# PaddlePaddle/PaddleNLP

Measured on NVIDIA H100. Metric: tokens/sec Llama-3.2-3B seq4096 bf16 pretrain step (global, all GPUs), higher is better.
Workload: dtype bf16

## Files before the change

### paddlenlp_b200/csrc/common.cuh

```cuda
#pragma once
#include <cuda.h>
#include <cuda_bf16.h>
#include <cuda_runtime.h>
#include <stdint.h>
#include <stdio.h>

namespace b200 {

typedef __nv_bfloat16 bf16;

__device__ __forceinline__ uint32_t smem_u32(const void* p) {
  return static_cast<uint32_t>(__cvta_generic_to_shared(p));
}
__device__ __forceinline__ void named_bar_sync(uint32_t id, uint32_t nthreads) {
  asm volatile("bar.sync %0, %1;" ::"r"(id), "r"(nthreads) : "memory");
}

__device__ __forceinline__ void pdl_wait() { asm volatile("griddepcontrol.wait;" ::: "memory"); }
__device__ __forceinline__ void pdl_launch_dependents() { asm volatile("griddepcontrol.launch_dependents;" ::: "memory"); }

__device__ __forceinline__ void mbar_init(uint64_t* bar, uint32_t count) {
  asm volatile("mbarrier.init.shared::cta.b64 [%0], %1;" ::"r"(smem_u32(bar)), "r"(count) : "memory");
}
__device__ __forceinline__ void fence_mbar_init() {
// ... 59 lines not shown
                                            int c2, int c3) {
  asm volatile(
      "cp.async.bulk.tensor.4d.shared::cluster.global.mbarrier::complete_tx::bytes [%0], [%1, {%3, %4, %5, %6}], [%2];"
      ::"r"(smem_u32(smem_dst)), "l"(reinterpret_cast<uint64_t>(tm)), "r"(smem_u32(bar)), "r"(c0), "r"(c1), "r"(c2),
      "r"(c3)
      : "memory");
}
__device__ __forceinline__ void tma_reduce_add_4d(const CUtensorMap* tm, const void* smem_src, int c0, int c1, int c2,
                                                  int c3) {
  asm volatile("cp.reduce.async.bulk.tensor.4d.global.shared::cta.add.tile.bulk_group [%0, {%2, %3, %4, %5}], [%1];" ::"l"(
                   reinterpret_cast<uint64_t>(tm)),
               "r"(smem_u32(smem_src)), "r"(c0), "r"(c1), "r"(c2), "r"(c3)
               : "memory");
}
__device__ __forceinline__ void tma_reduce_add_2d(const CUtensorMap* tm, uint32_t smem_src, int c0, int c1) {
  asm volatile("cp.reduce.async.bulk.tensor.2d.global.shared::cta.add.tile.bulk_group [%0, {%2, %3}], [%1];" ::"l"(
                   reinterpret_cast<uint64_t>(tm)),
               "r"(smem_src), "r"(c0), "r"(c1)
               : "memory");
}
__device__ __forceinline__ void tma_store_2d(const CUtensorMap* tm, uint32_t smem_src, int c0, int c1) {
  asm volatile("cp.async.bulk.tensor.2d.global.shared::cta.bulk_group [%0, {%2, %3}], [%1];" ::"l"(reinterpret_cast<uint64_t>(tm)),
               "r"(smem_src), "r"(c0), "r"(c1)
               : "memory");
}
__device__ __forceinline__ void tma_prefetch_l2_2d(const CUtensorMap* tm, int c0, int c1) {
  asm volatile("cp.async.bulk.prefetch.tensor.2d.L2.global.tile [%0, {%1, %2}];" ::"l"(reinterpret_cast<uint64_t>(tm)), "r"(c0),
               "r"(c1)
               : "memory");
}
__device__ __forceinline__ void tma_store_commit() { asm volatile("cp.async.bulk.commit_group;" ::: "memory"); }
template <int N>
__device__ __forceinline__ void tma_store_wait_read() {
  asm volatile("cp.async.bulk.wait_group.read %0;" ::"n"(N) : "memory");
}
template <int N>
__device__ __forceinline__ void tma_store_wait() {
  asm volatile("cp.async.bulk.wait_group %0;" ::"n"(N) : "memory");
}

__device__ __forceinline__ uint64_t wgmma_desc_sw128(uint32_t saddr, uint32_t lbo_bytes, uint32_t sbo_bytes) {
  uint64_t d = 0;
  d |= static_cast<uint64_t>((saddr & 0x3FFFFu) >> 4);
  d |= static_cast<uint64_t>((lbo_bytes >> 4) & 0x3FFFu) << 16;
  d |= static_cast<uint64_t>((sbo_bytes >> 4) & 0x3FFFu) << 32;
  d |= static_cast<uint64_t>(1) << 62;
  return d;
}
__device__ __forceinline__ void wgmma_fence() { asm volatile("wgmma.fence.sync.aligned;" ::: "memory"); }
__device__ __forceinline__ void wgmma_commit() { asm volatile("wgmma.commit_group.sync.aligned;" ::: "memory"); }
template <int N>
__device__ __forceinline__ void wgmma_wait() { asm volatile("wgmma.wait_group.sync.aligned %0;" ::"n"(N) : "memory"); }
template <int R>
__device__ __forceinline__ void setmaxnreg_dec() { asm volatile("setmaxnreg.dec.sync.aligned.u32 %0;" ::"n"(R)); }
template <int R>
__device__ __forceinline__ void setmaxnreg_inc() { asm volatile("setmaxnreg.inc.sync.aligned.u32 %0;" ::"n"(R)); }

template <int TA, int TB>
__device__ __forceinline__ void wgmma_m64n256k16(float (&d)[128], uint64_t desc_a, uint64_t desc_b, uint32_t accumulate) {
  asm volatile(
      "{\n\t.reg .pred p;\n\tsetp.ne.b32 p, %130, 0;\n\t"
      "wgmma.mma_async.sync.aligned.m64n256k16.f32.bf16.bf16 "
      "{%0, %1, %2, %3, %4, %5, %6, %7, %8, %9, %10, %11, %12, %13, %14, %15, %16, %17, %18, %19, %20, %21, %22, %23, %24, %25, %26, %27, %28, %29, %30, %31, %32, %33, %34, %35, %36, %37, %38, %39, %40, %41, %42, %43, %44, %45, %46, %47, %48, %49, %50, %51, %52, %53, %54, %55, %56, %57, %58, %59, %60, %61, %62, %63, %64, %65, %66, %67, %68, %69, %70, %71, %72, %73, %74, %75, %76, %77, %78, %79, %80, %81, %82, %83, %84, %85, %86, %87, %88, %89, %90, %91, %92, %93, %94, %95, %96, %97, %98, %99, %100, %101, %102, %103, %104, %105, %106, %107, %108, %109, %110, %111, %112, %113, %114, %115, %116, %117, %118, %119, %120, %121, %122, %123, %124, %125, %126, %127}, %128, %129, p, 1, 1, %131, %132;\n\t}\n"
      : "+f"(d[0]), "+f"(d[1]), "+f"(d[2]), "+f"(d[3]), "+f"(d[4]), "+f"(d[5]), "+f"(d[6]), "+f"(d[7]), "+f"(d[8]), "+f"(d[9]), "+f"(d[10]), "+f"(d[11]), "+f"(d[12]), "+f"(d[13]), "+f"(d[14]), "+f"(d[15]), "+f"(d[16]), "+f"(d[17]), "+f"(d[18]), "+f"(d[19]), "+f"(d[20]), "+f"(d[21]), "+f"(d[22]), "+f"(d[23]), "+f"(d[24]), "+f"(d[25]), "+f"(d[26]), "+f"(d[27]), "+f"(d[28]), "+f"(d[29]), "+f"(d[30]), "+f"(d[31]), "+f"(d[32]), "+f"(d[33]), "+f"(d[34]), "+f"(d[35]), "+f"(d[36]), "+f"(d[37]), "+f"(d[38]), "+f"(d[39]), "+f"(d[40]), "+f"(d[41]), "+f"(d[42]), "+f"(d[43]), "+f"(d[44]), "+f"(d[45]), "+f"(d[46]), "+f"(d[47]), "+f"(d[48]), "+f"(d[49]), "+f"(d[50]), "+f"(d[51]), "+f"(d[52]), "+f"(d[53]), "+f"(d[54]), "+f"(d[55]), "+f"(d[56]), "+f"(d[57]), "+f"(d[58]), "+f"(d[59]), "+f"(d[60]), "+f"(d[61]), "+f"(d[62]), "+f"(d[63]), "+f"(d[64]), "+f"(d[65]), "+f"(d[66]), "+f"(d[67]), "+f"(d[68]), "+f"(d[69]), "+f"(d[70]), "+f"(d[71]), "+f"(d[72]), "+f"(d[73]), "+f"(d[74]), "+f"(d[75]), "+f"(d[76]), "+f"(d[77]), "+f"(d[78]), "+f"(d[79]), "+f"(d[80]), "+f"(d[81]), "+f"(d[82]), "+f"(d[83]), "+f"(d[84]), "+f"(d[85]), "+f"(d[86]), "+f"(d[87]), "+f"(d[88]), "+f"(d[89]), "+f"(d[90]), "+f"(d[91]), "+f"(d[92]), "+f"(d[93]), "+f"(d[94]), "+f"(d[95]), "+f"(d[96]), "+f"(d[97]), "+f"(d[98]), "+f"(d[99]), "+f"(d[100]), "+f"(d[101]), "+f"(d[102]), "+f"(d[103]), "+f"(d[104]), "+f"(d[105]), "+f"(d[106]), "+f"(d[107]), "+f"(d[108]), "+f"(d[109]), "+f"(d[110]), "+f"(d[111]), "+f"(d[112]), "+f"(d[113]), "+f"(d[114]), "+f"(d[115]), "+f"(d[116]), "+f"(d[117]), "+f"(d[118]), "+f"(d[119]), "+f"(d[120]), "+f"(d[121]), "+f"(d[122]), "+f"(d[123]), "+f"(d[124]), "+f"(d[125]), "+f"(d[126]), "+f"(d[127])
      : "l"(desc_a), "l"(desc_b), "r"(accumulate), "n"(TA), "n"(TB));
}
template <int TA, int TB>
__device__ __forceinline__ void wgmma_m64n64k16(float (&d)[32], uint64_t desc_a, uint64_t desc_b, uint32_t accumulate) {
  asm volatile(
      "{\n\t.reg .pred p;\n\tsetp.ne.b32 p, %34, 0;\n\t"
      "wgmma.mma_async.sync.aligned.m64n64k16.f32.bf16.bf16 "
      "{%0, %1, %2, %3, %4, %5, %6, %7, %8, %9, %10, %11, %12, %13, %14, %15, %16, %17, %18, %19, %20, %21, %22, %23, %24, %25, %26, %27, %28, %29, %30, %31}, %32, %33, p, 1, 1, %35, %36;\n\t}\n"
      : "+f"(d[0]), "+f"(d[1]), "+f"(d[2]), "+f"(d[3]), "+f"(d[4]), "+f"(d[5]), "+f"(d[6]), "+f"(d[7]), "+f"(d[8]), "+f"(d[9]), "+f"(d[10]), "+f"(d[11]), "+f"(d[12]), "+f"(d[13]), "+f"(d[14]), "+f"(d[15]), "+f"(d[16]), "+f"(d[17]), "+f"(d[18]), "+f"(d[19]), "+f"(d[20]), "+f"(d[21]), "+f"(d[22]), "+f"(d[23]), "+f"(d[24]), "+f"(d[25]), "+f"(d[26]), "+f"(d[27]), "+f"(d[28]), "+f"(d[29]), "+f"(d[30]), "+f"(d[31])
      : "l"(desc_a), "l"(desc_b), "r"(accumulate), "n"(TA), "n"(TB));
}
template <int TA, int TB>
__device__ __forceinline__ void wgmma_m64n128k16(float (&d)[64], uint64_t desc_a, uint64_t desc_b, uint32_t accumulate) {
  asm volatile(
      "{\n\t.reg .pred p;\n\tsetp.ne.b32 p, %66, 0;\n\t"
      "wgmma.mma_async.sync.aligned.m64n128k16.f32.bf16.bf16 "
      "{%0, %1, %2, %3, %4, %5, %6, %7, %8, %9, %10, %11, %12, %13, %14, %15, %16, %17, %18, %19, %20, %21, %22, %23, %24, %25, %26, %27, %28, %29, %30, %31, %32, %33, %34, %35, %36, %37, %38, %39, %40, %41, %42, %43, %44, %45, %46, %47, %48, %49, %50, %51, %52, %53, %54, %55, %56, %57, %58, %59, %60, %61, %62, %63}, %64, %65, p, 1, 1, %67, %68;\n\t}\n"
      : "+f"(d[0]), "+f"(d[1]), "+f"(d[2]), "+f"(d[3]), "+f"(d[4]), "+f"(d[5]), "+f"(d[6]), "+f"(d[7]), "+f"(d[8]), "+f"(d[9]), "+f"(d[10]), "+f"(d[11]), "+f"(d[12]), "+f"(d[13]), "+f"(d[14]), "+f"(d[15]), "+f"(d[16]), "+f"(d[17]), "+f"(d[18]), "+f"(d[19]), "+f"(d[20]), "+f"(d[21]), "+f"(d[22]), "+f"(d[23]), "+f"(d[24]), "+f"(d[25]), "+f"(d[26]), "+f"(d[27]), "+f"(d[28]), "+f"(d[29]), "+f"(d[30]), "+f"(d[31]), "+f"(d[32]), "+f"(d[33]), "+f"(d[34]), "+f"(d[35]), "+f"(d[36]), "+f"(d[37]), "+f"(d[38]), "+f"(d[39]), "+f"(d[40]), "+f"(d[41]), "+f"(d[42]), "+f"(d[43]), "+f"(d[44]), "+f"(d[45]), "+f"(d[46]), "+f"(d[47]), "+f"(d[48]), "+f"(d[49]), "+f"(d[50]), "+f"(d[51]), "+f"(d[52]), "+f"(d[53]), "+f"(d[54]), "+f"(d[55]), "+f"(d[56]), "+f"(d[57]), "+f"(d[58]), "+f"(d[59]), "+f"(d[60]), "+f"(d[61]), "+f"(d[62]), "+f"(d[63])
      : "l"(desc_a), "l"(desc_b), "r"(accumulate), "n"(TA), "n"(TB));
}
template <int TB>
__device__ __forceinline__ void wgmma_m64n128k16_rs(float (&d)[64], const uint32_t* a, uint64_t desc_b, uint32_t accumulate) {
  asm volatile(
      "{\n\t.reg .pred p;\n\tsetp.ne.b32 p, %69, 0;\n\t"
      "wgmma.mma_async.sync.aligned.m64n128k16.f32.bf16.bf16 "
      "{%0, %1, %2, %3, %4, %5, %6, %7, %8, %9, %10, %11, %12, %13, %14, %15, %16, %17, %18, %19, %20, %21, %22, %23, %24, %25, %26, %27, %28, %29, %30, %31, %32, %33, %34, %35, %36, %37, %38, %39, %40, %41, %42, %43, %44, %45, %46, %47, %48, %49, %50, %51, %52, %53, %54, %55, %56, %57, %58, %59, %60, %61, %62, %63}, {%64, %65, %66, %67}, %68, p, 1, 1, %70;\n\t}\n"
      : "+f"(d[0]), "+f"(d[1]), "+f"(d[2]), "+f"(d[3]), "+f"(d[4]), "+f"(d[5]), "+f"(d[6]), "+f"(d[7]), "+f"(d[8]), "+f"(d[9]), "+f"(d[10]), "+f"(d[11]), "+f"(d[12]), "+f"(d[13]), "+f"(d[14]), "+f"(d[15]), "+f"(d[16]), "+f"(d[17]), "+f"(d[18]), "+f"(d[19]), "+f"(d[20]), "+f"(d[21]), "+f"(d[22]), "+f"(d[23]), "+f"(d[24]), "+f"(d[25]), "+f"(d[26]), "+f"(d[27]), "+f"(d[28]), "+f"(d[29]), "+f"(d[30]), "+f"(d[31]), "+f"(d[32]), "+f"(d[33]), "+f"(d[34]), "+f"(d[35]), "+f"(d[36]), "+f"(d[37]), "+f"(d[38]), "+f"(d[39]), "+f"(d[40]), "+f"(d[41]), "+f"(d[42]), "+f"(d[43]), "+f"(d[44]), "+f"(d[45]), "+f"(d[46]), "+f"(d[47]), "+f"(d[48]), "+f"(d[49]), "+f"(d[50]), "+f"(d[51]), "+f"(d[52]), "+f"(d[53]), "+f"(d[54]), "+f"(d[55]), "+f"(d[56]), "+f"(d[57]), "+f"(d[58]), "+f"(d[59]), "+f"(d[60]), "+f"(d[61]), "+f"(d[62]), "+f"(d[63])
      : "r"(a[0]), "r"(a[1]), "r"(a[2]), "r"(a[3]), "l"(desc_b), "r"(accumulate), "n"(TB));
}
template <int TB>
__device__ __forceinline__ void wgmma_m64n64k16_rs(float (&d)[32], const uint32_t* a, uint64_t desc_b, uint32_t accumulate) {
  asm volatile(
      "{\n\t.reg .pred p;\n\tsetp.ne.b32 p, %37, 0;\n\t"
      "wgmma.mma_async.sync.aligned.m64n64k16.f32.bf16.bf16 "
      "{%0, %1, %2, %3, %4, %5, %6, %7, %8, %9, %10, %11, %12, %13, %14, %15, %16, %17, %18, %19, %20, %21, %22, %23, %24, %25, %26, %27, %28, %29, %30, %31}, {%32, %33, %34, %35}, %36, p, 1, 1, %38;\n\t}\n"
      : "+f"(d[0]), "+f"(d[1]), "+f"(d[2]), "+f"(d[3]), "+f"(d[4]), "+f"(d[5]), "+f"(d[6]), "+f"(d[7]), "+f"(d[8]), "+f"(d[9]), "+f"(d[10]), "+f"(d[11]), "+f"(d[12]), "+f"(d[13]), "+f"(d[14]), "+f"(d[15]), "+f"(d[16]), "+f"(d[17]), "+f"(d[18]), "+f"(d[19]), "+f"(d[20]), "+f"(d[21]), "+f"(d[22]), "+f"(d[23]), "+f"(d[24]), "+f"(d[25]), "+f"(d[26]), "+f"(d[27]), "+f"(d[28]), "+f"(d[29]), "+f"(d[30]), "+f"(d[31])
      : "r"(a[0]), "r"(a[1]), "r"(a[2]), "r"(a[3]), "l"(desc_b), "r"(accumulate), "n"(TB));
}

__device__ __forceinline__ void mma_bf16_16816(float (&c)[4], const uint32_t (&a)[4], uint32_t b0, uint32_t b1) {
  asm volatile(
      "mma.sync.aligned.m16n8k16.row.col.f32.bf16.bf16.f32 {%0, %1, %2, %3}, {%4, %5, %6, %7}, {%8, %9}, "
      "{%0, %1, %2, %3};"
      : "+f"(c[0]), "+f"(c[1]), "+f"(c[2]), "+f"(c[3])
      : "r"(a[0]), "r"(a[1]), "r"(a[2]), "r"(a[3]), "r"(b0), "r"(b1));
}
__device__ __forceinline__ void ldsm_x4(uint32_t saddr, uint32_t (&r)[4]) {
  asm volatile("ldmatrix.sync.aligned.m8n8.x4.shared.b16 {%0, %1, %2, %3}, [%4];"
               : "=r"(r[0]), "=r"(r[1]), "=r"(r[2]), "=r"(r[3])
               : "r"(saddr));
}
__device__ __forceinline__ void ldsm_x4_t(uint32_t saddr, uint32_t (&r)[4]) {
  asm volatile("ldmatrix.sync.aligned.m8n8.x4.trans.shared.b16 {%0, %1, %2, %3}, [%4];"
               : "=r"(r[0]), "=r"(r[1]), "=r"(r[2]), "=r"(r[3])
               : "r"(saddr));
}
__device__ __forceinline__ void cp_async_16(uint32_t saddr, const void* gptr, uint32_t src_bytes) {
  asm volatile("cp.async.cg.shared.global [%0], [%1], 16, %2;" ::"r"(saddr), "l"(gptr), "r"(src_bytes) : "memory");
}
__device__ __forceinline__ void cp_async_commit() { asm volatile("cp.async.commit_group;" ::: "memory"); }
template <int N>
__device__ __forceinline__ void cp_async_wait() { asm volatile("cp.async.wait_group %0;" ::"n"(N) : "memory"); }

__device__ __forceinline__ uint32_t pack_bf16x2(float lo, float hi) {
  __nv_bfloat162 v = __floats2bfloat162_rn(lo, hi);
  return *reinterpret_cast<uint32_t*>(&v);
}
__device__ __forceinline__ float2 unpack_bf16x2(uint32_t u) {
  __nv_bfloat162 v = *reinterpret_cast<__nv_bfloat162*>(&u);
  return __bfloat1622float2(v);
}
__device__ __forceinline__ float bf16_round(float x) { return __bfloat162float(__float2bfloat16_rn(x)); }

__device__ __forceinline__ uint4 ld_nc_v4(const void* p) {
  uint4 r;
  asm("ld.global.nc.L1::no_allocate.v4.u32 {%0, %1, %2, %3}, [%4];"
               : "=r"(r.x), "=r"(r.y), "=r"(r.z), "=r"(r.w)
               : "l"(p));
  return r;
}
__device__ __forceinline__ void st_na_v4(void* p, const uint4& v) {
  asm volatile("st.global.L1::no_allocate.v4.u32 [%0], {%1, %2, %3, %4};" ::"l"(p), "r"(v.x), "r"(v.y), "r"(v.z),
               "r"(v.w));
}
__device__ __forceinline__ void st_shared_u32(uint32_t saddr, uint32_t v) {
  asm volatile("st.shared.u32 [%0], %1;" ::"r"(saddr), "r"(v));
}
__device__ __forceinline__ void st_shared_f32x2(uint32_t saddr, float a, float b) {
  asm volatile("st.shared.v2.f32 [%0], {%1, %2};" ::"r"(saddr), "f"(a), "f"(b));
}
__device__ __forceinline__ uint4 ld_shared_v4(uint32_t saddr) {
  uint4 r;
  asm volatile("ld.shared.v4.u32 {%0, %1, %2, %3}, [%4];" : "=r"(r.x), "=r"(r.y), "=r"(r.z), "=r"(r.w) : "r"(saddr));
  return r;
}

__device__ __forceinline__ float fast_exp2(float x) {
  float y;
  asm("ex2.approx.ftz.f32 %0, %1;" : "=f"(y) : "f"(x));
  return y;
}
__device__ __forceinline__ float fast_rcp(float x) {
  float y;
  asm("rcp.approx.ftz.f32 %0, %1;" : "=f"(y) : "f"(x));
  return y;
}

struct f32x2 { float x, y; };
__device__ __forceinline__ f32x2 f2_mul(f32x2 a, f32x2 b) { return f32x2{__fmul_rn(a.x, b.x), __fmul_rn(a.y, b.y)}; }
__device__ __forceinline__ f32x2 f2_add(f32x2 a, f32x2 b) { return f32x2{__fadd_rn(a.x, b.x), __fadd_rn(a.y, b.y)}; }
__device__ __forceinline__ f32x2 f2_fma(f32x2 a, f32x2 b, f32x2 c) {
  return f32x2{__fmaf_rn(a.x, b.x, c.x), __fmaf_rn(a.y, b.y, c.y)};
}

__device__ __forceinline__ uint32_t swiglu_fwd_pair(uint32_t g2, uint32_t u2) {
  const float2 gf = unpack_bf16x2(g2), uf = unpack_bf16x2(u2);
  const f32x2 g{gf.x, gf.y}, u{uf.x, uf.y}, one{1.f, 1.f};
  const f32x2 t = f2_mul(g, f32x2{-1.4426950408889634f, -1.4426950408889634f});
  const f32x2 a = f2_add(f32x2{fast_exp2(t.x), fast_exp2(t.y)}, one);
  const f32x2 sg{fast_rcp(a.x), fast_rcp(a.y)};
  const f32x2 m = f2_mul(f2_mul(g, sg), u);
  return pack_bf16x2(m.x, m.y);
}

__device__ __forceinline__ void swiglu_bwd_pair(uint32_t g2, uint32_t u2, float d0, float d1, uint32_t& dg2, uint32_t& du2) {
  const float2 gf = unpack_bf16x2(g2), uf = unpack_bf16x2(u2);
  const f32x2 g{gf.x, gf.y}, u{uf.x, uf.y}, d{d0, d1}, one{1.f, 1.f};
  const f32x2 t = f2_mul(g, f32x2{-1.4426950408889634f, -1.4426950408889634f});
  const f32x2 a = f2_add(f32x2{fast_exp2(t.x), fast_exp2(t.y)}, one);
  const f32x2 sg{fast_rcp(a.x), fast_rcp(a.y)};
  const f32x2 silu = f2_mul(g, sg);
  const f32x2 om = f2_fma(sg, f32x2{-1.f, -1.f}, one);
  const f32x2 ds = f2_mul(sg, f2_fma(g, om, one));
  const f32x2 dgv = f2_mul(f2_mul(d, u), ds);
  const f32x2 duv = f2_mul(d, silu);
  dg2 = pack_bf16x2(dgv.x, dgv.y);
  du2 = pack_bf16x2(duv.x, duv.y);
}

template <bool FUSE_SIN = false>
__device__ __forceinline__ void rope_rotate_chunk(uint4& a, uint4& b, const float* cos_t, const float* sin_t, int pos, int half,
                                                  int j8, float sign = 1.f) {
  const float4* c4 = reinterpret_cast<const float4*>(cos_t + static_cast<size_t>(pos) * half + j8);
  const float4* s4 = reinterpret_cast<const float4*>(sin_t + static_cast<size_t>(pos) * half + j8);
  const float4 c0 = __ldg(c4), c1 = __ldg(c4 + 1), s0 = __ldg(s4), s1 = __ldg(s4 + 1);
  const float cs[8] = {c0.x, c0.y, c0.z, c0.w, c1.x, c1.y, c1.z, c1.w};
  const float sn[8] = {s0.x, s0.y, s0.z, s0.w, s1.x, s1.y, s1.z, s1.w};
  uint32_t* ai = reinterpret_cast<uint32_t*>(&a);
  uint32_t* bi = reinterpret_cast<uint32_t*>(&b);
  auto first = [](float x1, float x2, float c, float s) { return __fmaf_rn(x1, c, -__fmul_rn(x2, s)); };
  auto second = [](float x1, float x2, float c, float s) {
    return FUSE_SIN ? __fmaf_rn(x1, s, __fmul_rn(x2, c)) : __fmaf_rn(x2, c, __fmul_rn(x1, s));
  };
#pragma unroll
  for (int j = 0; j < 4; ++j) {
    const float2 x1 = unpack_bf16x2(ai[j]), x2 = unpack_bf16x2(bi[j]);
    const float s_lo = sign * sn[2 * j], s_hi = sign * sn[2 * j + 1];
    ai[j] = pack_bf16x2(first(x1.x, x2.x, cs[2 * j], s_lo), first(x1.y, x2.y, cs[2 * j + 1], s_hi));
    bi[j] = pack_bf16x2(second(x1.x, x2.x, cs[2 * j], s_lo), second(x1.y, x2.y, cs[2 * j + 1], s_hi));
  }
}

__device__ __forceinline__ float warp_sum(float v) {
#pragma unroll
  for (int o = 16; o > 0; o >>= 1) v += __shfl_xor_sync(0xffffffffu, v, o);
  return v;
}

constexpr int DECODE_PART_ROW = 132;
constexpr int DECODE_PART_M = 128;

}
```

### paddlenlp_b200/csrc/gemm_wgmma.cu

```cuda
#include "../../include/b200nlp.h"
#include <cstdlib>
#include <cstring>

#include "common.cuh"
#include "host_util.h"

namespace b200 {
namespace gemm {

constexpr int BN = 256;
constexpr int BK = 64;
constexpr int B_BYTES = BN * BK * 2;
constexpr int EPI_BOX = 64;
constexpr int EPI_BOX_BYTES = EPI_BOX * EPI_BOX * 2;
constexpr int EPI_BOX_F32 = 32;

template <int NWG>
struct Tile {
  static constexpr int BM = 64 * NWG;
  static constexpr int NUM_THREADS = 128 * (NWG + 1);
  static constexpr int A_BYTES = BM * BK * 2;
  static constexpr int STAGE_BYTES = A_BYTES + B_BYTES;
  static constexpr int STAGES = NWG == 2 ? 4 : 5;
  static constexpr int EPI_BYTES = NWG * 2 * EPI_BOX_BYTES;
  static constexpr int SMEM_BYTES = STAGES * STAGE_BYTES + EPI_BYTES + 256 + 1024;
};
static int tile_wgs(int64_t M) { return M <= 64 ? 1 : 2; }

struct Params {
  int M, N, K;
  int num_m_tiles, num_n_tiles;
  int epi_mode;
  int swiglu_inter;
  int gm;
  int split_k;
  int kb_per_split;
  const float* bias;
  bf16* c;
  int64_t ldc;
  const bf16* r;
  int64_t ldr;
  bf16* aux;
  int64_t ld_aux;
  float* ws;
};

__device__ __forceinline__ void tile_coords(int t, int num_m, int num_n, int& m_blk, int& n_blk, int GM) {
  const int per_group = GM * num_n;
  const int g = t / per_group;
  const int first_m = g * GM;
  const int gsize = min(GM, num_m - first_m);
  const int r = t - g * per_group;
  m_blk = first_m + (r % gsize);
  n_blk = r / gsize;
}

__device__ __forceinline__ void fence_acc(float (&acc)[128]) {
#pragma unroll
  for (int i = 0; i < 128; ++i) asm volatile("" : "+f"(acc[i])::"memory");
}

__device__ __forceinline__ uint32_t epi_slot(uint32_t buf, int r, int jj, int lane) {
  return buf + r * 128 + ((jj ^ (r & 7)) << 4) + 4 * (lane & 3);
}
template <int KEEP>
__device__ __forceinline__ void epi_begin(int cw, bool leader) {
  if (leader) tma_store_wait_read<KEEP>();
  named_bar_sync(1 + cw, 128);
}
__device__ __forceinline__ void epi_end(int cw) {
  fence_proxy_async_smem();
  named_bar_sync(1 + cw, 128);
}
__device__ __forceinline__ uint32_t ld_pair(const bf16* base, int64_t ld, int row, int col, int M, int N) {
  if (row >= M || col >= N) return 0u;
  const bf16* src = base + static_cast<int64_t>(row) * ld + col;
  if (col + 1 < N) return *reinterpret_cast<const uint32_t*>(src);
  return static_cast<uint32_t>(__bfloat16_as_ushort(*src));
}
__device__ __forceinline__ void epi_prefetch(const CUtensorMap* tmC, const CUtensorMap* tmX, const Params& p, int n_blk, int row0) {
  for (int s = 0; s < BN / EPI_BOX; ++s) {
    const int col0 = n_blk * BN + EPI_BOX * s;
    if (col0 >= p.N) break;
    if (p.epi_mode == 1) {
      tma_prefetch_l2_2d(tmC, col0, row0);
    } else if (p.epi_mode == 2) {
      tma_prefetch_l2_2d(tmX, col0, row0);
    } else {
      tma_prefetch_l2_2d(tmX, col0, row0);
      tma_prefetch_l2_2d(tmX, p.swiglu_inter + col0, row0);
    }
  }
}

template <int NWG, bool A_MN, bool B_MN>
__global__ void __launch_bounds__(Tile<NWG>::NUM_THREADS, 1)
gemm_bf16_kernel(const __grid_constant__ CUtensorMap tmA, const __grid_constant__ CUtensorMap tmB,
                 const __grid_constant__ CUtensorMap tmC, const __grid_constant__ CUtensorMap tmX, const Params p) {
  using T = Tile<NWG>;
  constexpr int BM = T::BM, A_BYTES = T::A_BYTES, STAGE_BYTES = T::STAGE_BYTES, STAGES = T::STAGES;
  extern __shared__ uint8_t smem_raw[];
  uint8_t* smem = reinterpret_cast<uint8_t*>((reinterpret_cast<uintptr_t>(smem_raw) + 1023) & ~uintptr_t(1023));
  uint64_t* full_bar = reinterpret_cast<uint64_t*>(smem + STAGES * STAGE_BYTES + T::EPI_BYTES);
  uint64_t* empty_bar = full_bar + STAGES;

  const int num_items = p.num_m_tiles * p.num_n_tiles * p.split_k;
  const int num_kb_total = (p.K + BK - 1) / BK;
  if (threadIdx.x == 0) {
    tma_prefetch_desc(&tmA);
    tma_prefetch_desc(&tmB);
    for (int i = 0; i < STAGES; ++i) {
      mbar_init(&full_bar[i], 1);
      mbar_init(&empty_bar[i], NWG * 128);
    }
    fence_mbar_init();
  }
  __syncthreads();
  pdl_launch_dependents();
  pdl_wait();

  const int wg = threadIdx.x >> 7;
  if (wg == 0) {
    setmaxnreg_dec<40>();
    if (threadIdx.x == 0) {
      uint32_t it = 0;
      for (int t = blockIdx.x; t < num_items; t += gridDim.x) {
        int m_blk, n_blk;
        tile_coords(t / p.split_k, p.num_m_tiles, p.num_n_tiles, m_blk, n_blk, p.gm);
        const int kb0 = (t % p.split_k) * p.kb_per_split;
        const int kb1 = min(num_kb_total, kb0 + p.kb_per_split);
        for (int kb = kb0; kb < kb1; ++kb, ++it) {
          const int st = static_cast<int>(it % STAGES);
          mbar_wait_nocall(&empty_bar[st], ((it / STAGES) & 1u) ^ 1u);
          uint8_t* sA = smem + st * STAGE_BYTES;
          uint8_t* sB = sA + A_BYTES;
          mbar_arrive_expect_tx(&full_bar[st], STAGE_BYTES);
          if constexpr (A_MN) {
#pragma unroll
            for (int h = 0; h < NWG; ++h) tma_load_2d(&tmA, &full_bar[st], sA + h * (64 * BK * 2), m_blk * BM + 64 * h, kb * BK);
          } else {
            tma_load_2d(&tmA, &full_bar[st], sA, kb * BK, m_blk * BM);
          }
          if constexpr (B_MN) {
#pragma unroll
            for (int h = 0; h < 4; ++h) {
              const int c0 = p.epi_mode == 4 ? (h >> 1) * p.swiglu_inter + n_blk * 128 + (h & 1) * 64 : n_blk * BN + h * 64;
              tma_load_2d(&tmB, &full_bar[st], sB + h * (B_BYTES / 4), c0, kb * BK);
            }
          } else {
            tma_load_2d(&tmB, &full_bar[st], sB, kb * BK, n_blk * BN);
            tma_load_2d(&tmB, &full_bar[st], sB + B_BYTES / 2, kb * BK, n_blk * BN + 128);
          }
        }
      }
    }
    return;
  }

  setmaxnreg_inc<232>();
  const int cw = wg - 1;
  const int wi = (threadIdx.x >> 5) & 3, lane = threadIdx.x & 31;
  const uint32_t ring = smem_u32(smem);
  constexpr uint32_t A_KSTEP = A_MN ? 2048u : 32u, B_KSTEP = B_MN ? 2048u : 32u;
  const uint32_t a_off = static_cast<uint32_t>(cw) * (64 * BK * 2);
  const bool leader = (threadIdx.x & 127) == 0;
  const bool prefetch = leader && (p.epi_mode == 1 || p.epi_mode == 2 || p.epi_mode == 5);
  const uint32_t ebuf = smem_u32(smem + STAGES * STAGE_BYTES) + cw * 2 * EPI_BOX_BYTES;
  uint32_t nbox = 0;
  uint32_t it = 0;
  float acc[128];
  for (int t = blockIdx.x; t < num_items; t += gridDim.x) {
    int m_blk, n_blk;
    tile_coords(t / p.split_k, p.num_m_tiles, p.num_n_tiles, m_blk, n_blk, p.gm);
    const int kb0 = (t % p.split_k) * p.kb_per_split;
    const int nkb = min(num_kb_total, kb0 + p.kb_per_split) - kb0;
    const int prefetch_kb = nkb > 8 ? nkb - 8 : 0;
    fence_acc(acc);
#pragma unroll
    for (int i = 0; i < 128; ++i) acc[i] = 0.f;
    fence_acc(acc);
    for (int i = 0; i < nkb; ++i, ++it) {
      const int st = static_cast<int>(it % STAGES);
      mbar_wait_nocall(&full_bar[st], (it / STAGES) & 1u);
      const uint32_t sA = ring + st * STAGE_BYTES + a_off, sB = ring + st * STAGE_BYTES + A_BYTES;
      const uint64_t dA = wgmma_desc_sw128(sA, A_MN ? 64 * BK * 2 : 16, 1024);
      const uint64_t dB = wgmma_desc_sw128(sB, B_MN ? B_BYTES / 4 : 16, 1024);
      wgmma_fence();
#pragma unroll
      for (int kk = 0; kk < BK / 16; ++kk)
        wgmma_m64n256k16<A_MN ? 1 : 0, B_MN ? 1 : 0>(acc, dA + ((kk * A_KSTEP) >> 4), dB + ((kk * B_KSTEP) >> 4),
                                                     (i > 0 || kk > 0) ? 1u : 0u);
      wgmma_commit();
      if (prefetch && i == prefetch_kb) epi_prefetch(&tmC, &tmX, p, n_blk, m_blk * BM + cw * 64);
      wgmma_wait<1>();
      if (i > 0) mbar_arrive(&empty_bar[(it - 1) % STAGES]);
    }
    wgmma_wait<0>();
    fence_acc(acc);
    if (nkb > 0) mbar_arrive(&empty_bar[(it - 1) % STAGES]);

    const int row0 = m_blk * BM + cw * 64;
    const int r_lo = wi * 16 + (lane >> 2);
    const int cq = 2 * (lane & 3);
    if (p.epi_mode == 3) {
#pragma unroll
      for (int i = 0; i < 2; ++i) {
        const int row = row0 + r_lo + 8 * i;
        if (row >= p.M) continue;
#pragma unroll
        for (int j = 0; j < 32; ++j) {
          const int col = n_blk * BN + 8 * j + cq;
          if (col >= p.N) continue;
          float* w = p.ws + static_cast<int64_t>(row) * p.N + col;
          asm volatile("red.global.add.v2.f32 [%0], {%1, %2};" ::"l"(w), "f"(acc[4 * j + 2 * i]), "f"(acc[4 * j + 2 * i + 1])
                       : "memory");
        }
      }
      continue;
    }
    if (p.epi_mode == 4) {
#pragma unroll
      for (int h = 0; h < 2; ++h) {
        const int ch0 = n_blk * 128 + EPI_BOX * h;
        if (ch0 >= p.swiglu_inter) continue;
        if (p.aux != nullptr) {
          epi_begin<0>(cw, leader);
#pragma unroll
          for (int i = 0; i < 2; ++i)
#pragma unroll
            for (int jj = 0; jj < 8; ++jj) {
              const int j = 8 * h + jj;
              st_shared_u32(epi_slot(ebuf, r_lo + 8 * i, jj, lane), pack_bf16x2(acc[4 * j + 2 * i], acc[4 * j + 2 * i + 1]));
              st_shared_u32(epi_slot(ebuf + EPI_BOX_BYTES, r_lo + 8 * i, jj, lane),
                            pack_bf16x2(acc[4 * (j + 16) + 2 * i], acc[4 * (j + 16) + 2 * i + 1]));
            }
          epi_end(cw);
          if (leader) {
            tma_store_2d(&tmX, ebuf, ch0, row0);
            tma_store_2d(&tmX, ebuf + EPI_BOX_BYTES, p.swiglu_inter + ch0, row0);
            tma_store_commit();
          }
        }
        epi_begin<0>(cw, leader);
#pragma unroll
        for (int i = 0; i < 2; ++i)
#pragma unroll
          for (int jj = 0; jj < 8; ++jj) {
            const int j = 8 * h + jj;
            const uint32_t gp = pack_bf16x2(acc[4 * j + 2 * i], acc[4 * j + 2 * i + 1]);
            const uint32_t up = pack_bf16x2(acc[4 * (j + 16) + 2 * i], acc[4 * (j + 16) + 2 * i + 1]);
            st_shared_u32(epi_slot(ebuf, r_lo + 8 * i, jj, lane), swiglu_fwd_pair(gp, up));
          }
        epi_end(cw);
        if (leader) {
          tma_store_2d(&tmC, ebuf, ch0, row0);
          tma_store_commit();
        }
      }
      continue;
    }
    if (p.epi_mode == 5) {
#pragma unroll
      for (int s = 0; s < BN / EPI_BOX; ++s) {
        const int ch0 = n_blk * BN + EPI_BOX * s;
        if (ch0 >= p.N) continue;
        epi_begin<0>(cw, leader);
#pragma unroll
        for (int q = 0; q < 4; ++q) {
          const int i = q >> 1, jj0 = 4 * (q & 1);
          uint32_t g[4], u[4];
#pragma unroll
          for (int k = 0; k < 4; ++k) {
            const int row = row0 + r_lo + 8 * i, ch = ch0 + 8 * (jj0 + k) + cq;
            g[k] = ld_pair(p.aux, p.ld_aux, row, ch, p.M, p.N);
            u[k] = ld_pair(p.aux + p.swiglu_inter, p.ld_aux, row, ch, p.M, p.N);
          }
#pragma unroll
          for (int k = 0; k < 4; ++k) {
            const int jj = jj0 + k, j = 8 * s + jj;
            uint32_t dg2, du2;
            swiglu_bwd_pair(g[k], u[k], bf16_round(acc[4 * j + 2 * i]), bf16_round(acc[4 * j + 2 * i + 1]), dg2, du2);
            st_shared_u32(epi_slot(ebuf, r_lo + 8 * i, jj, lane), dg2);
            st_shared_u32(epi_slot(ebuf + EPI_BOX_BYTES, r_lo + 8 * i, jj, lane), du2);
          }
        }
        epi_end(cw);
        if (leader) {
          tma_store_2d(&tmC, ebuf, ch0, row0);
          tma_store_2d(&tmC, ebuf + EPI_BOX_BYTES, p.swiglu_inter + ch0, row0);
          tma_store_commit();
        }
      }
      continue;
    }
#pragma unroll
    for (int s = 0; s < BN / EPI_BOX; ++s) {
      const int col0 = n_blk * BN + EPI_BOX * s;
      if (col0 >= p.N) continue;
      if (p.epi_mode >= 6) {
        const uint32_t sw = (lane >> 2) << 4;
        const uint32_t row_off = r_lo * 128 + ((8 * (lane & 3)) ^ (sw & 16));
        epi_begin<0>(cw, leader);
#pragma unroll
        for (int h = 0; h < 2; ++h)
#pragma unroll
          for (int jj = 0; jj < 4; ++jj) {
            const int j = 8 * s + 4 * h + jj;
            const uint32_t slot = ebuf + h * EPI_BOX_BYTES + row_off + ((32 * jj) ^ (sw & 96));
            st_shared_f32x2(slot, acc[4 * j], acc[4 * j + 1]);
            st_shared_f32x2(slot + 8 * 128, acc[4 * j + 2], acc[4 * j + 3]);
          }
        epi_end(cw);
        if (leader) {
          if (p.epi_mode == 7) {
            tma_reduce_add_2d(&tmC, ebuf, col0, row0);
            tma_reduce_add_2d(&tmC, ebuf + EPI_BOX_BYTES, col0 + EPI_BOX_F32, row0);
          } else {
            tma_store_2d(&tmC, ebuf, col0, row0);
            tma_store_2d(&tmC, ebuf + EPI_BOX_BYTES, col0 + EPI_BOX_F32, row0);
          }
          tma_store_commit();
        }
        continue;
      }
      const uint32_t buf = ebuf + (nbox++ & 1u) * EPI_BOX_BYTES;
      epi_begin<1>(cw, leader);
#pragma unroll
      for (int i = 0; i < 2; ++i) {
        uint32_t o[8];
        if (p.epi_mode != 0) {
          const bf16* src = p.epi_mode == 1 ? p.c : p.r;
          const int64_t ld = p.epi_mode == 1 ? p.ldc : p.ldr;
#pragma unroll
          for (int jj = 0; jj < 8; ++jj) o[jj] = ld_pair(src, ld, row0 + r_lo + 8 * i, col0 + 8 * jj + cq, p.M, p.N);
        }
#pragma unroll
        for (int jj = 0; jj < 8; ++jj) {
          const int j = 8 * s + jj, col = col0 + 8 * jj + cq;
          float f0 = acc[4 * j + 2 * i], f1 = acc[4 * j + 2 * i + 1];
          if (p.bias != nullptr) {
            if (col < p.N) f0 += __ldg(p.bias + col);
            if (col + 1 < p.N) f1 += __ldg(p.bias + col + 1);
          }
          if (p.epi_mode != 0) {
            if (p.epi_mode == 2) { f0 = bf16_round(f0); f1 = bf16_round(f1); }
            const float2 of = unpack_bf16x2(o[jj]);
            f0 += of.x;
            f1 += of.y;
          }
          st_shared_u32(epi_slot(buf, r_lo + 8 * i, jj, lane), pack_bf16x2(f0, f1));
        }
      }
      epi_end(cw);
      if (leader) {
        tma_store_2d(&tmC, buf, col0, row0);
        tma_store_commit();
      }
    }
  }
  if (leader) tma_store_wait<0>();
}

template <int NWG, bool A_MN, bool B_MN>
static int launch(const CUtensorMap& tmA, const CUtensorMap& tmB, const CUtensorMap& tmC, const CUtensorMap& tmX, const Params& p,
                  int max_ctas, cudaStream_t stream) {
  using T = Tile<NWG>;
  constexpr int SMEM_BYTES = T::SMEM_BYTES;
  auto kern = gemm_bf16_kernel<NWG, A_MN, B_MN>;
  static bool attr_set = false;
  if (!attr_set) {
    cudaError_t e = cudaFuncSetAttribute(kern, cudaFuncAttributeMaxDynamicSharedMemorySize, SMEM_BYTES);
    if (e != cudaSuccess) {
      set_last_error("cudaFuncSetAttribute(gemm smem=%d): %s", SMEM_BYTES, cudaGetErrorString(e));
      return static_cast<int>(e);
    }
    attr_set = true;
  }
  const int num_items = p.num_m_tiles * p.num_n_tiles * p.split_k;
  int ctas = sm_count();
  if (max_ctas > 0 && max_ctas < ctas) ctas = max_ctas;
  if (ctas > num_items) ctas = num_items;
  Params pp = p;
  pp.gm = (16ll * 128 * p.K * 2 <= (18ll << 20)) ? 16 : 8;
  cudaError_t e = launch_pdl(kern, dim3(ctas), dim3(T::NUM_THREADS), SMEM_BYTES, stream, tmA, tmB, tmC, tmX, pp);
  if (e != cudaSuccess) {
    set_last_error("gemm launch: %s", cudaGetErrorString(e));
    return static_cast<int>(e);
  }
  return 0;
}

static int make_epi_map(CUtensorMap* tm, const void* base, int64_t rows, int64_t cols, int64_t ld) {
  const uint64_t dims[2] = {static_cast<uint64_t>(cols), static_cast<uint64_t>(rows)}, strides[1] = {static_cast<uint64_t>(ld) * 2};
  const uint32_t box[2] = {EPI_BOX, EPI_BOX};
  return encode_tmap_bf16(tm, base, 2, dims, strides, box);
}
static int make_epi_map_f32(CUtensorMap* tm, const void* base, int64_t rows, int64_t cols, int64_t ld) {
  const uint64_t dims[2] = {static_cast<uint64_t>(cols), static_cast<uint64_t>(rows)}, strides[1] = {static_cast<uint64_t>(ld) * 4};
  const uint32_t box[2] = {EPI_BOX_F32, EPI_BOX};
  return encode_tmap_f32(tm, base, 2, dims, strides, box);
}
static bool aligned16(const void* ptr) { return (reinterpret_cast<uintptr_t>(ptr) & 15) == 0; }

static int setup_smem_epilogue(const Params& p, CUtensorMap* tmC, CUtensorMap* tmX) {
  int rc;
  switch (p.epi_mode) {
    case 2:
      if ((rc = make_epi_map(tmX, p.r, p.M, p.N, p.ldr)) != 0) return rc;
      return make_epi_map(tmC, p.c, p.M, p.N, p.ldc);
    case 3:
      return 0;
    case 6:
    case 7:
      return make_epi_map_f32(tmC, p.ws, p.M, p.N, p.ldc);
    case 4:
      if (p.aux != nullptr && (rc = make_epi_map(tmX, p.aux, p.M, p.N, p.ld_aux)) != 0) return rc;
      return make_epi_map(tmC, p.c, p.M, p.swiglu_inter, p.ldc);
    case 5:
      if ((rc = make_epi_map(tmX, p.aux, p.M, 2ll * p.N, p.ld_aux)) != 0) return rc;
      return make_epi_map(tmC, p.c, p.M, 2ll * p.N, p.ldc);
    default:
      return make_epi_map(tmC, p.c, p.M, p.N, p.ldc);
  }
}

static int dispatch(bool a_mn, bool b_mn, const CUtensorMap& tmA, const CUtensorMap& tmB, Params p, int max_ctas,
                    cudaStream_t stream) {
  CUtensorMap tmC, tmX;
  memset(&tmC, 0, sizeof(tmC));
  memset(&tmX, 0, sizeof(tmX));
  int rc;
  if ((rc = setup_smem_epilogue(p, &tmC, &tmX)) != 0) return rc;
  if (tile_wgs(p.M) == 1) {
    if (a_mn && b_mn) return launch<1, true, true>(tmA, tmB, tmC, tmX, p, max_ctas, stream);
    if (a_mn) return launch<1, true, false>(tmA, tmB, tmC, tmX, p, max_ctas, stream);
    if (b_mn) return launch<1, false, true>(tmA, tmB, tmC, tmX, p, max_ctas, stream);
    return launch<1, false, false>(tmA, tmB, tmC, tmX, p, max_ctas, stream);
  }
  if (a_mn && b_mn) return launch<2, true, true>(tmA, tmB, tmC, tmX, p, max_ctas, stream);
  if (a_mn) return launch<2, true, false>(tmA, tmB, tmC, tmX, p, max_ctas, stream);
  if (b_mn) return launch<2, false, true>(tmA, tmB, tmC, tmX, p, max_ctas, stream);
  return launch<2, false, false>(tmA, tmB, tmC, tmX, p, max_ctas, stream);
}

static int make_a_map(CUtensorMap* tm, const void* A, int64_t M, int64_t K, int64_t lda, bool mn) {
  uint64_t dims[2], strides[1] = {static_cast<uint64_t>(lda) * 2};
  uint32_t box[2];
  if (mn) { dims[0] = M; dims[1] = K; box[0] = 64; box[1] = BK; }
  else    { dims[0] = K; dims[1] = M; box[0] = BK; box[1] = 64 * tile_wgs(M); }
  return encode_tmap_bf16(tm, A, 2, dims, strides, box);
}
static int make_b_map(CUtensorMap* tm, const void* B, int64_t N, int64_t K, int64_t ldb, bool mn) {
  uint64_t dims[2], strides[1] = {static_cast<uint64_t>(ldb) * 2};
  uint32_t box[2];
  if (mn) { dims[0] = N; dims[1] = K; box[0] = 64; box[1] = BK; }
  else    { dims[0] = K; dims[1] = N; box[0] = BK; box[1] = 128; }
  return encode_tmap_bf16(tm, B, 2, dims, strides, box);
}

static Params base_params(int64_t M, int64_t N, int64_t K) {
  Params p = {};
  p.M = static_cast<int>(M);
  p.N = static_cast<int>(N);
  p.K = static_cast<int>(K);
  const int64_t bm = 64 * tile_wgs(M);
  p.num_m_tiles = static_cast<int>((M + bm - 1) / bm);
  p.num_n_tiles = static_cast<int>((N + BN - 1) / BN);
  p.split_k = 1;
  p.kb_per_split = static_cast<int>((K + BK - 1) / BK);
  return p;
}

}
}

extern "C" int b200_gemm_bf16_ex(const void* A, const void* B, void* C, const float* bias, const void* residual,
                                 int64_t M, int64_t N, int64_t K, int64_t lda, int64_t ldb, int64_t ldc, int64_t ldr,
                                 int a_mn_major, int b_mn_major, int accumulate, int max_ctas, cudaStream_t stream) {
  using namespace b200;
  using namespace b200::gemm;
  B200_CHECK_ARG(A && B && C, "gemm: null pointer");
  B200_CHECK_ARG(M > 0 && N > 0 && K > 0, "gemm: non-positive dimension M=%lld N=%lld K=%lld", (long long)M,
                 (long long)N, (long long)K);
  B200_CHECK_ARG(lda % 8 == 0 && ldb % 8 == 0 && ldc % 8 == 0, "gemm: leading dimensions must be multiples of 8");
  B200_CHECK_ARG(!(residual && accumulate), "gemm: residual and accumulate are mutually exclusive");
  B200_CHECK_ARG(!residual || ldr % 8 == 0, "gemm: ldr must be a multiple of 8");
  B200_CHECK_ARG(M < (1ll << 31) && N < (1ll << 31) && K < (1ll << 31), "gemm: dimension too large");
  B200_CHECK_ARG(aligned16(C), "gemm: C must be 16-byte aligned");
  B200_CHECK_ARG(!residual || aligned16(residual), "gemm: residual must be 16-byte aligned");
  CUtensorMap tmA, tmB;
  int rc;
  if ((rc = make_a_map(&tmA, A, M, K, lda, a_mn_major)) != 0) return rc;
  if ((rc = make_b_map(&tmB, B, N, K, ldb, b_mn_major)) != 0) return rc;
  Params p = base_params(M, N, K);
  p.epi_mode = residual ? 2 : (accumulate ? 1 : 0);
  p.bias = bias;
  p.c = static_cast<bf16*>(C);
  p.ldc = ldc;
  p.r = static_cast<const bf16*>(residual);
  p.ldr = ldr;
  return dispatch(a_mn_major, b_mn_major, tmA, tmB, p, max_ctas, stream);
}

extern "C" int b200_gemm_bf16_f32(const void* A, const void* B, float* C, int64_t M, int64_t N, int64_t K, int64_t lda,
                                  int64_t ldb, int64_t ldc, int a_mn_major, int b_mn_major, int accumulate, cudaStream_t stream) {
// ... 145 lines not shown
```

Measured before the change: 24300.

## Load GEMM epilogue inputs via TMA into shared memory instead of global loads

Replaces the per-thread global loads of epilogue operands (residual, accumulate-into C, SwiGLU gate/up aux) and the L2 prefetch with TMA 2D loads into the epilogue shared-memory boxes, tracked by new per-warpgroup mbarriers. The first box is issued during the tail of the K loop, and later boxes are double-buffered ahead of use. Threads then read the operand from the swizzled smem slot and overwrite it in place with the output before the TMA store. This is meant to remove scattered uncoalesced global loads and latency from the epilogue. In exchange it adds barrier phase tracking and waits on store-read completion before reusing buffers, so a phase mismatch could cause hangs or wrong results.

Result: faster. 24940 (median of 6 runs) (+2.7%).

```diff
diff --git a/paddlenlp_b200/csrc/common.cuh b/paddlenlp_b200/csrc/common.cuh
--- a/paddlenlp_b200/csrc/common.cuh
+++ b/paddlenlp_b200/csrc/common.cuh
@@ -235,6 +235,11 @@
 }
 __device__ __forceinline__ void st_shared_f32x2(uint32_t saddr, float a, float b) {
   asm volatile("st.shared.v2.f32 [%0], {%1, %2};" ::"r"(saddr), "f"(a), "f"(b));
+}
+__device__ __forceinline__ uint32_t ld_shared_u32(uint32_t saddr) {
+  uint32_t r;
+  asm volatile("ld.shared.u32 %0, [%1];" : "=r"(r) : "r"(saddr));
+  return r;
 }
 __device__ __forceinline__ uint4 ld_shared_v4(uint32_t saddr) {
   uint4 r;
diff --git a/paddlenlp_b200/csrc/gemm_wgmma.cu b/paddlenlp_b200/csrc/gemm_wgmma.cu
--- a/paddlenlp_b200/csrc/gemm_wgmma.cu
+++ b/paddlenlp_b200/csrc/gemm_wgmma.cu
@@ -24,6 +24,7 @@
   static constexpr int STAGES = NWG == 2 ? 4 : 5;
   static constexpr int EPI_BYTES = NWG * 2 * EPI_BOX_BYTES;
   static constexpr int SMEM_BYTES = STAGES * STAGE_BYTES + EPI_BYTES + 256 + 1024;
+  static_assert((2 * STAGES + 2 * NWG) * 8 <= 256, "barrier area");
 };
 static int tile_wgs(int64_t M) { return M <= 64 ? 1 : 2; }
 
@@ -72,25 +73,26 @@
   fence_proxy_async_smem();
   named_bar_sync(1 + cw, 128);
 }
-__device__ __forceinline__ uint32_t ld_pair(const bf16* base, int64_t ld, int row, int col, int M, int N) {
-  if (row >= M || col >= N) return 0u;
-  const bf16* src = base + static_cast<int64_t>(row) * ld + col;
-  if (col + 1 < N) return *reinterpret_cast<const uint32_t*>(src);
-  return static_cast<uint32_t>(__bfloat16_as_ushort(*src));
-}
-__device__ __forceinline__ void epi_prefetch(const CUtensorMap* tmC, const CUtensorMap* tmX, const Params& p, int n_blk, int row0) {
-  for (int s = 0; s < BN / EPI_BOX; ++s) {
-    const int col0 = n_blk * BN + EPI_BOX * s;
-    if (col0 >= p.N) break;
-    if (p.epi_mode == 1) {
-      tma_prefetch_l2_2d(tmC, col0, row0);
-    } else if (p.epi_mode == 2) {
-      tma_prefetch_l2_2d(tmX, col0, row0);
-    } else {
-      tma_prefetch_l2_2d(tmX, col0, row0);
-      tma_prefetch_l2_2d(tmX, p.swiglu_inter + col0, row0);
-    }
-  }
+__device__ __forceinline__ void epi_load(const CUtensorMap* tm, uint64_t* bar, uint8_t* buf, int col, int row) {
+  mbar_arrive_expect_tx(bar, EPI_BOX_BYTES);
+  tma_load_2d(tm, bar, buf, col, row);
+}
+__device__ __forceinline__ void epi_wait(uint64_t* bars, uint32_t b, uint32_t& phase) {
+  mbar_wait_nocall(&bars[b], (phase >> b) & 1u);
+  phase ^= 1u << b;
+}
+__device__ __forceinline__ void epi_load_first(const CUtensorMap* tm, const Params& p, uint8_t* ebox, uint64_t* bars,
+                                               uint32_t nbox, int n_blk, int row0) {
+  const int col0 = n_blk * BN;
+  tma_store_wait_read<0>();
+  if (p.epi_mode == 5) {
+    epi_load(tm, &bars[0], ebox, col0, row0);
+    epi_load(tm, &bars[1], ebox + EPI_BOX_BYTES, p.swiglu_inter + col0, row0);
+    return;
+  }
+  const uint32_t b = nbox & 1u;
+  epi_load(tm, &bars[b], ebox + b * EPI_BOX_BYTES, col0, row0);
+  if (col0 + EPI_BOX < p.N) epi_load(tm, &bars[b ^ 1u], ebox + (b ^ 1u) * EPI_BOX_BYTES, col0 + EPI_BOX, row0);
 }
 
 template <int NWG, bool A_MN, bool B_MN>
@@ -103,6 +105,7 @@
   uint8_t* smem = reinterpret_cast<uint8_t*>((reinterpret_cast<uintptr_t>(smem_raw) + 1023) & ~uintptr_t(1023));
   uint64_t* full_bar = reinterpret_cast<uint64_t*>(smem + STAGES * STAGE_BYTES + T::EPI_BYTES);
   uint64_t* empty_bar = full_bar + STAGES;
+  uint64_t* epi_bar = empty_bar + STAGES;
 
   const int num_items = p.num_m_tiles * p.num_n_tiles * p.split_k;
   const int num_kb_total = (p.K + BK - 1) / BK;
@@ -113,6 +116,7 @@
       mbar_init(&full_bar[i], 1);
       mbar_init(&empty_bar[i], NWG * 128);
     }
+    for (int i = 0; i < 2 * NWG; ++i) mbar_init(&epi_bar[i], 1);
     fence_mbar_init();
   }
   __syncthreads();
@@ -164,9 +168,13 @@
   constexpr uint32_t A_KSTEP = A_MN ? 2048u : 32u, B_KSTEP = B_MN ? 2048u : 32u;
   const uint32_t a_off = static_cast<uint32_t>(cw) * (64 * BK * 2);
   const bool leader = (threadIdx.x & 127) == 0;
-  const bool prefetch = leader && (p.epi_mode == 1 || p.epi_mode == 2 || p.epi_mode == 5);
-  const uint32_t ebuf = smem_u32(smem + STAGES * STAGE_BYTES) + cw * 2 * EPI_BOX_BYTES;
+  const bool has_input = p.epi_mode == 1 || p.epi_mode == 2 || p.epi_mode == 5;
+  uint8_t* const ebox = smem + STAGES * STAGE_BYTES + cw * 2 * EPI_BOX_BYTES;
+  const uint32_t ebuf = smem_u32(ebox);
+  uint64_t* const ebar = epi_bar + 2 * cw;
+  const CUtensorMap* const tm_in = p.epi_mode == 1 ? &tmC : &tmX;
   uint32_t nbox = 0;
+  uint32_t ephase = 0;
   uint32_t it = 0;
   float acc[128];
   for (int t = blockIdx.x; t < num_items; t += gridDim.x) {
@@ -174,7 +182,7 @@
     tile_coords(t / p.split_k, p.num_m_tiles, p.num_n_tiles, m_blk, n_blk, p.gm);
     const int kb0 = (t % p.split_k) * p.kb_per_split;
     const int nkb = min(num_kb_total, kb0 + p.kb_per_split) - kb0;
-    const int prefetch_kb = nkb > 8 ? nkb - 8 : 0;
+    const int load_kb = nkb > 8 ? nkb - 8 : 0;
     fence_acc(acc);
 #pragma unroll
     for (int i = 0; i < 128; ++i) acc[i] = 0.f;
@@ -191,7 +199,7 @@
         wgmma_m64n256k16<A_MN ? 1 : 0, B_MN ? 1 : 0>(acc, dA + ((kk * A_KSTEP) >> 4), dB + ((kk * B_KSTEP) >> 4),
                                                      (i > 0 || kk > 0) ? 1u : 0u);
       wgmma_commit();
-      if (prefetch && i == prefetch_kb) epi_prefetch(&tmC, &tmX, p, n_blk, m_blk * BM + cw * 64);
+      if (leader && has_input && i == load_kb) epi_load_first(tm_in, p, ebox, ebar, nbox, n_blk, m_blk * BM + cw * 64);
       wgmma_wait<1>();
       if (i > 0) mbar_arrive(&empty_bar[(it - 1) % STAGES]);
     }
@@ -264,26 +272,25 @@
       for (int s = 0; s < BN / EPI_BOX; ++s) {
         const int ch0 = n_blk * BN + EPI_BOX * s;
         if (ch0 >= p.N) continue;
-        epi_begin<0>(cw, leader);
-#pragma unroll
-        for (int q = 0; q < 4; ++q) {
-          const int i = q >> 1, jj0 = 4 * (q & 1);
-          uint32_t g[4], u[4];
-#pragma unroll
-          for (int k = 0; k < 4; ++k) {
-            const int row = row0 + r_lo + 8 * i, ch = ch0 + 8 * (jj0 + k) + cq;
-            g[k] = ld_pair(p.aux, p.ld_aux, row, ch, p.M, p.N);
-            u[k] = ld_pair(p.aux + p.swiglu_inter, p.ld_aux, row, ch, p.M, p.N);
-          }
-#pragma unroll
-          for (int k = 0; k < 4; ++k) {
-            const int jj = jj0 + k, j = 8 * s + jj;
+        if (s > 0 && leader) {
+          tma_store_wait_read<0>();
+          epi_load(tm_in, &ebar[0], ebox, ch0, row0);
+          epi_load(tm_in, &ebar[1], ebox + EPI_BOX_BYTES, p.swiglu_inter + ch0, row0);
+        }
+        epi_wait(ebar, 0, ephase);
+        epi_wait(ebar, 1, ephase);
+#pragma unroll
+        for (int i = 0; i < 2; ++i)
+#pragma unroll
+          for (int jj = 0; jj < 8; ++jj) {
+            const int j = 8 * s + jj;
+            const uint32_t sg = epi_slot(ebuf, r_lo + 8 * i, jj, lane), su = sg + EPI_BOX_BYTES;
             uint32_t dg2, du2;
-            swiglu_bwd_pair(g[k], u[k], bf16_round(acc[4 * j + 2 * i]), bf16_round(acc[4 * j + 2 * i + 1]), dg2, du2);
-            st_shared_u32(epi_slot(ebuf, r_lo + 8 * i, jj, lane), dg2);
-            st_shared_u32(epi_slot(ebuf + EPI_BOX_BYTES, r_lo + 8 * i, jj, lane), du2);
-          }
-        }
+            swiglu_bwd_pair(ld_shared_u32(sg), ld_shared_u32(su), bf16_round(acc[4 * j + 2 * i]),
+                            bf16_round(acc[4 * j + 2 * i + 1]), dg2, du2);
+            st_shared_u32(sg, dg2);
+            st_shared_u32(su, du2);
+          }
         epi_end(cw);
         if (leader) {
           tma_store_2d(&tmC, ebuf, ch0, row0);
@@ -323,20 +330,22 @@
         }
         continue;
       }
-      const uint32_t buf = ebuf + (nbox++ & 1u) * EPI_BOX_BYTES;
-      epi_begin<1>(cw, leader);
-#pragma unroll
-      for (int i = 0; i < 2; ++i) {
-        uint32_t o[8];
-        if (p.epi_mode != 0) {
-          const bf16* src = p.epi_mode == 1 ? p.c : p.r;
-          const int64_t ld = p.epi_mode == 1 ? p.ldc : p.ldr;
-#pragma unroll
-          for (int jj = 0; jj < 8; ++jj) o[jj] = ld_pair(src, ld, row0 + r_lo + 8 * i, col0 + 8 * jj + cq, p.M, p.N);
-        }
+      const uint32_t b = nbox++ & 1u, buf = ebuf + b * EPI_BOX_BYTES;
+      if (p.epi_mode == 0) {
+        epi_begin<1>(cw, leader);
+      } else {
+        if (s > 0 && s + 1 < BN / EPI_BOX && col0 + EPI_BOX < p.N && leader) {
+          tma_store_wait_read<0>();
+          epi_load(tm_in, &ebar[b ^ 1u], ebox + (b ^ 1u) * EPI_BOX_BYTES, col0 + EPI_BOX, row0);
+        }
+        epi_wait(ebar, b, ephase);
+      }
+#pragma unroll
+      for (int i = 0; i < 2; ++i)
 #pragma unroll
         for (int jj = 0; jj < 8; ++jj) {
           const int j = 8 * s + jj, col = col0 + 8 * jj + cq;
+          const uint32_t slot = epi_slot(buf, r_lo + 8 * i, jj, lane);
           float f0 = acc[4 * j + 2 * i], f1 = acc[4 * j + 2 * i + 1];
           if (p.bias != nullptr) {
             if (col < p.N) f0 += __ldg(p.bias + col);
@@ -344,13 +353,12 @@
           }
           if (p.epi_mode != 0) {
             if (p.epi_mode == 2) { f0 = bf16_round(f0); f1 = bf16_round(f1); }
-            const float2 of = unpack_bf16x2(o[jj]);
+            const float2 of = unpack_bf16x2(ld_shared_u32(slot));
             f0 += of.x;
             f1 += of.y;
           }
-          st_shared_u32(epi_slot(buf, r_lo + 8 * i, jj, lane), pack_bf16x2(f0, f1));
-        }
-      }
+          st_shared_u32(slot, pack_bf16x2(f0, f1));
+        }
       epi_end(cw);
       if (leader) {
         tma_store_2d(&tmC, buf, col0, row0);
```
